# antoine311200/sow

Measured on AMD Instinct MI355X. Metric: SoWLinear fwd+bwd tokens/s, llama_60m rank=50 (56-layer SoWLinear stack), higher is better.
Workload: dtype bf16

## Files before the change

### sow_amd/csrc/api.hip

```cpp
#include "kernels.hpp"
#include <cstring>
#include <vector>
#include <cstdio>
#include <cstdlib>

namespace sow {

template <typename T, typename TO>
__global__ __launch_bounds__(256) void colsum_kernel(const T* M, int64_t ld, int64_t rows, int D, TO* out, float beta) {
  __shared__ float red[4][64];
  const int c = blockIdx.x * 64 + (threadIdx.x & 63), w = threadIdx.x >> 6;
  float s = 0.f;
  if (c < D)
    for (int64_t i = w; i < rows; i += 4) s += to_f32(M[i * ld + c]);
  red[w][threadIdx.x & 63] = s;
  __syncthreads();
  if (w == 0 && c < D) {
    float v = red[0][threadIdx.x] + red[1][threadIdx.x] + red[2][threadIdx.x] + red[3][threadIdx.x];
    if (beta != 0.f) v += beta * to_f32(out[c]);
    out[c] = from_f32<TO>(v);
  }
}
static int launch_colsum(const void* dy, int64_t T, int d_out, void* dbias, float beta, int dtype, int out_dtype,
                         hipStream_t stream) {
  const dim3 grid((d_out + 63) / 64);
  if (out_dtype != dtype && out_dtype != SOW_F32) return SOW_ERR_DTYPE;
  const bool o32 = out_dtype == SOW_F32;
  if (dtype == SOW_F32)
    hipLaunchKernelGGL((colsum_kernel<float, float>), grid, dim3(256), 0, stream, (const float*)dy, (int64_t)d_out, T, d_out, (float*)dbias, beta);
  else if (dtype == SOW_BF16 && o32)
    hipLaunchKernelGGL((colsum_kernel<bf16_t, float>), grid, dim3(256), 0, stream, (const bf16_t*)dy, (int64_t)d_out, T, d_out, (float*)dbias, beta);
  else if (dtype == SOW_BF16)
    hipLaunchKernelGGL((colsum_kernel<bf16_t, bf16_t>), grid, dim3(256), 0, stream, (const bf16_t*)dy, (int64_t)d_out, T, d_out, (bf16_t*)dbias, beta);
  else if (dtype == SOW_F16 && o32)
    hipLaunchKernelGGL((colsum_kernel<f16_t, float>), grid, dim3(256), 0, stream, (const f16_t*)dy, (int64_t)d_out, T, d_out, (float*)dbias, beta);
  else if (dtype == SOW_F16)
    hipLaunchKernelGGL((colsum_kernel<f16_t, f16_t>), grid, dim3(256), 0, stream, (const f16_t*)dy, (int64_t)d_out, T, d_out, (f16_t*)dbias, beta);
  else
    return SOW_ERR_DTYPE;
  SOW_CHECK_LAUNCH();
  return SOW_OK;
}
}

namespace sow {
static const char* const kSwitchNames[SW_COUNT] = {"FORCE_CHAIN_V1", "NO_SHORT_SPLIT", "NO_FUSED_H", "FORCE_GEMM_V1", "TN_NARROW",
                                                   "NO_GEMM3S",      "GEMM3S",         "GEMM3",      "NO_GROUPED",     "NO_PERSIST",     "NO_NT_STORE",    "NT_LOAD",        "NO_PAIR_FLUSH",  "F32_EXACT",
                                                   "NO_PARK16",      "TN_NO_NT_LOAD",  "NO_TN_ROWS",     "GEMM4",          "NO_GEMM4H",      "NO_CHAIN3F",     "NO_TN_F32Q",     "NO_SPLITK",
                                                   "NO_WIDE_CHAIN",  "NO_SHARED_X",    "NO_RAGGED",      "NO_RAGGED_GEMM", "NO_BLOCKED_QR",
                                                   "NO_SKINNY",      "NO_FUSED_ACC",   "NO_DEEP_ACC",    "NO_F16_TN",
                                                   "NO_ROW_ALIGN",   "NO_X_PAIR",      "NO_H_ROWS"};
static std::atomic<int> g_switch[SW_COUNT];
static std::once_flag g_switch_once;
static void switches_from_env() {
  for (int i = 0; i < SW_COUNT; ++i) {
    char name[64];
    snprintf(name, sizeof name, "SOW_AMD_%s", kSwitchNames[i]);
    const char* v = getenv(name);
    const bool tri = i == SW_GEMM3S || i == SW_GEMM3 || i == SW_GEMM4;
    const int on = i == SW_NO_ROW_ALIGN && v && v[0] >= '1' && v[0] <= '3' ? v[0] - '0' : 1;
    g_switch[i].store(!v ? -1 : (tri ? (v[0] != '0') : on), std::memory_order_relaxed);
  }
}
int sw(int which) {
  std::call_once(g_switch_once, switches_from_env);
  return g_switch[which].load(std::memory_order_relaxed);
}
}

using namespace sow;

static inline size_t al256(size_t v) { return (v + 255) & ~(size_t)255; }
static inline size_t esize(int dtype) { return dtype == SOW_F32 ? 4 : 2; }
static inline bool ok_dtype(int d) { return d == SOW_F32 || d == SOW_BF16 || d == SOW_F16; }
struct Dtype {
  int cd;
  bool param_f32;
  bool fuse;
  bool deep;
  bool native;
  bool native_bit;
  int perm() const { return (fuse ? SOW_FUSE_ACC : 0) | (deep ? SOW_FUSE_ACC_DEEP : 0); }
  bool layer_ok() const { return ok_dtype(cd) && !((param_f32 || native_bit) && cd == SOW_F32); }
};
static inline Dtype decode_dtype(int d) {
  Dtype f;
  f.cd = d & ~(SOW_FUSE_ACC | SOW_FUSE_ACC_DEEP | SOW_PARAM_F32 | SOW_ACC_NATIVE);
  f.param_f32 = (d & SOW_PARAM_F32) != 0;
  f.native_bit = (d & SOW_ACC_NATIVE) != 0;
  f.native = f.native_bit && f.param_f32;
  f.fuse = (d & SOW_FUSE_ACC) != 0 && !f.param_f32;
  f.deep = (d & SOW_FUSE_ACC_DEEP) != 0 && !f.param_f32;
  return f;
}
static inline bool flagged(int d) { return (d & (SOW_PARAM_F32 | SOW_ACC_NATIVE)) != 0; }
static inline int nofuse(int d) { return d & ~(SOW_FUSE_ACC | SOW_FUSE_ACC_DEEP); }

constexpr int SHORT_NTB = 128;
static inline int short_want(int ntb) { return ntb > 0 ? (256 + ntb - 1) / ntb : 1; }
static size_t short_hp_bytes(int64_t T, int d_in, int d_out, int r_live, int dtype) {
  const int ntb = ceil_div(T, 64);
  if (r_live > 64 || ntb <= 0 || ntb > SHORT_NTB) return 0;
  const int dmax = d_in > d_out ? d_in : d_out;
  int ks = short_want(ntb);
// ... 1529 lines not shown
```

### sow_amd/csrc/chain2.hip

```cpp
#include "kernels.hpp"
#include "lds_dma.hpp"

namespace sow {

#ifdef SOW_STAMPS
#define C2_STAMP(i)                                                                                  \
  do {                                                                                               \
    if (stamps && w == 0 && lane == 0) stamps[i] = __builtin_amdgcn_s_memrealtime();                \
  } while (0)
#else
#define C2_STAMP(i) \
  do {              \
  } while (0)
#endif
#ifdef SOW_STAMPS
#define C2_TICK() __builtin_amdgcn_s_memrealtime()
#define C2_ACC(var, t0) var += __builtin_amdgcn_s_memrealtime() - (t0)
#define C2_PUT(cond, i, var)                     \
  do {                                           \
    if (stamps && (cond) && lane == 0) stamps[i] = (var); \
  } while (0)
#else
#define C2_TICK() 0ull
#define C2_ACC(var, t0) (void)(t0)
#define C2_PUT(cond, i, var) \
  do {                       \
  } while (0)
#endif

constexpr int C2_NTG = 2;
constexpr int C2_NCW = 2 * C2_NTG;
constexpr int C2_NLW = 2;
constexpr int C2_BM = 32 * C2_NTG;
#ifndef C2_DEPTH_X
#define C2_DEPTH_X 4
#define C2_NSLOT_X 6
#define C2_AHEAD_X 5
#endif
constexpr int C2_DEPTH = C2_DEPTH_X;
constexpr int C2_STAGE = 4096;
constexpr int C2_NSLOT = C2_NSLOT_X;
constexpr int C2_AHEAD = C2_AHEAD_X;
#ifdef C2_EXPERIMENT_SHALLOW_X
static_assert(C2_NSLOT == C2_AHEAD + 1 && C2_NSLOT + C2_DEPTH == 10 && C2_DEPTH >= 3 && C2_DEPTH <= 6, "80 KiB");
#else
static_assert(C2_NSLOT == C2_AHEAD + 1 && C2_NSLOT + C2_DEPTH == 10 && C2_DEPTH >= 4 && C2_DEPTH <= 6,
              "80 KiB: 8 KiB per chunk slot + 2 x 4 KiB per X slot; two 8-KiB fp32 park tiles per token group must fit its X ring");
#endif
constexpr int C2_FSLOT = 8192;
constexpr int C2_LPW = 8 / C2_NLW;
constexpr int C2_RING0 = C2_NSLOT * C2_FSLOT;
constexpr int C2_RING = C2_DEPTH * C2_STAGE;
constexpr int C2_LDS = C2_RING0 + C2_NTG * C2_RING;
constexpr int C2_THREADS = 64 * (C2_NCW + C2_NLW);
constexpr int C2_RESIDENT = 512;


__host__ __device__ constexpr int c2_x_issued(int st, int nst, int depth, bool paired) {
  const int n = paired ? depth - 2 + 2 * ((st + 1) >> 1) : depth - 1 + st;
  return n < nst ? n : nst;
}

template <bool TR> __device__ __forceinline__ int img_chunk(int row, int c) {
  return TR ? (c ^ (((row >> 1) & 1) << 2)) : (c ^ ((row >> 1) & 7));
}

template <typename T, bool BWD, bool P16, bool AL>
__device__ __forceinline__ void chain2_block(const ChainParams& p, const int bid, char* smem, const int t, const int lane, const int w,
                                             uint64_t* stamps) {
  constexpr bool TR = !BWD;
  C2_STAMP(0);
  const int tb = p.ntb > 0 ? bid % p.ntb : bid;
  const int split = p.ntb > 0 ? bid / p.ntb : 0;
  const int64_t m0 = (int64_t)tb * C2_BM;
  const int D1 = p.D1, D2 = p.D2, rb = p.rb;
  const int nst_all = (D1 + 63) / 64, nsl_all = (D2 + 63) / 64;
  const int st0 = p.st_per > 0 ? split * p.st_per : 0;
  const int sl0 = p.sl_per > 0 ? split * p.sl_per : 0;
  const int nst = p.sl_per > 0 ? 0 : (p.st_per > 0 ? (nst_all - st0 < p.st_per ? nst_all - st0 : p.st_per) : nst_all);
  const int nsl = p.st_per > 0 ? 0 : (p.sl_per > 0 ? (nsl_all - sl0 < p.sl_per ? nsl_all - sl0 : p.sl_per) : nsl_all);
  const int total = nst + nsl;
  const T* Amat = (const T*)(BWD ? p.F2b : p.F1b);
  const T* Bmat = (const T*)(BWD ? p.F1b : p.F2b);
  const int64_t ldb = BWD ? p.ldf1b : p.ldf2b;
  const int rows_a = BWD ? D2 : D1, cols_b = BWD ? D1 : D2;
  const char* zp = zero_page_for(lane);
  const int ral = AL ? p.row_align : 0;

  if (w >= C2_NCW) {
    __builtin_amdgcn_s_setprio(3);
    const int lw = w - C2_NCW;
    const char* a_end = (const char*)(Amat + (int64_t)rows_a * rb);
    const bool own_last = rows_a > 0 && lw == ((rows_a - 1) & 63) / (8 * C2_LPW);
    uint32_t last_row_dw = 0u;
    if (own_last && lane < 32 && 2 * lane < rb) last_row_dw = *((const uint32_t*)(Amat + (int64_t)(rows_a - 1) * rb) + lane);
    asm volatile("" : "+v"(last_row_dw));
    auto chunk_is_a = [&](int c) { return BWD ? (c >= nst) : (c < nst); };
    const char* a_ptr[C2_LPW];
    const char* b_ptr[C2_LPW];
    int b_stride[C2_LPW], b_lc[C2_LPW];
#pragma unroll
    for (int ii = 0; ii < C2_LPW; ++ii) {
      const int i = C2_LPW * lw + ii;
      const int row = 8 * i + (lane >> 3), pc = lane & 7;
      const int lc = img_chunk<TR>(row, pc);
      a_ptr[ii] = (const char*)(Amat + (int64_t)row * rb) + 16 * lc;
      const bool bv = row < rb;
      b_ptr[ii] = bv ? (const char*)(Bmat + (int64_t)row * ldb + 8 * lc) : zp;
      b_stride[ii] = bv ? 128 : 0;
      b_lc[ii] = lc;
    }
    const int a_chunk_bytes = 128 * rb;
    const bool b_ragged = (cols_b & 63) != 0;
    const int nb_chunks = (cols_b + 63) / 64;
    auto issue = [&](int c) {
#ifdef C2_EXPERIMENT_NO_FACTOR_DMA
      if (c >= C2_NSLOT) return;
#endif
#ifdef C2_EXPERIMENT_HALF_FACTOR_DMA
      if (bid & 1) return;
#endif
      char* slot = smem + (c % C2_NSLOT) * C2_FSLOT;
      const int ci = c < nst ? st0 + c : sl0 + (c - nst);
      if (chunk_is_a(c)) {
#pragma unroll
        for (int ii = 0; ii < C2_LPW; ++ii) {
          const char* q = a_ptr[ii] + (int64_t)ci * a_chunk_bytes;
          dma16(q + 16 <= a_end ? (const void*)q : (const void*)zp, slot + (C2_LPW * lw + ii) * 1024);
        }
      } else {
#pragma unroll
        for (int ii = 0; ii < C2_LPW; ++ii) {
          const char* q = b_ptr[ii] + ci * b_stride[ii];
          if (b_ragged && ci == nb_chunks - 1 && ci * 64 + 8 * b_lc[ii] >= cols_b) q = zp;
          dma16((const void*)q, slot + (C2_LPW * lw + ii) * 1024);
        }
      }
    };
    const int ahead = ral ? C2_AHEAD - 1 : C2_AHEAD;
    const int pre = total < ahead ? total : ahead;
    for (int c = 0; c < pre; ++c) issue(c);
    uint64_t tw_dma = 0, tw_bar = 0;
    for (int c = 0; c < total; ++c) {
      const int newer = (total - 1 - c) < (ahead - 1) ? (total - 1 - c) : (ahead - 1);
      const uint64_t tk0 = C2_TICK();
      wait_groups<C2_LPW>(newer);
      C2_ACC(tw_dma, tk0);
      if (chunk_is_a(c)) {
        const int base = (c < nst ? st0 + c : sl0 + (c - nst)) * 64;
        const int lr = rows_a - 1 - base;
        if (own_last && lr >= 0 && lr < 64 && lane < 32) {
          const int cc = lane >> 2;
          *(uint32_t*)(smem + (c % C2_NSLOT) * C2_FSLOT + lr * 128 + img_chunk<TR>(lr, cc) * 16 + (lane & 3) * 4) = last_row_dw;
        }
      }
      if (c == nst) __builtin_amdgcn_s_setprio(0);
      if (c == nst) raw_barrier();
      const uint64_t tk1 = C2_TICK();
      raw_barrier();
      C2_ACC(tw_bar, tk1);
      if (c + ahead < total) issue(c + ahead);
    }
    C2_PUT(w == C2_NCW, 8, tw_dma);
    C2_PUT(w == C2_NCW, 9, tw_bar);
    if (nsl > 0) {
      raw_barrier();
    } else {
      raw_barrier();
    }
    raw_barrier();
    return;
  }

  if (p.pad_dst && bid * 64 < p.pad_rows) {
    const T* src = (const T*)p.pad_src;
    T* dst = (T*)p.pad_dst;
#pragma unroll
    for (int it = 0; it < 2; ++it) {
      const int idx = t + 256 * it, row = bid * 64 + (idx >> 3), c0 = (idx & 7) * 8;
      if (row < p.pad_rows) {
        u32x4 v;
        T* e = (T*)&v;
#pragma unroll
        for (int j = 0; j < 8; ++j) e[j] = (c0 + j < p.pad_r) ? src[(int64_t)row * p.pad_r + c0 + j] : (T)0.f;
        *(u32x4*)(dst + (int64_t)row * 64 + c0) = v;
      }
    }
  }
  const int tg = w & 1, hh = w >> 1;
  const int li = lane & 31, lh = lane >> 5;
  const int g = lane >> 4, jj = lane & 15, q = jj >> 2, pp = jj & 3;
  const int h2 = g >> 1;
  char* ring = smem + C2_RING0 + tg * C2_RING;
  const uint32_t ring_a = lds_addr(ring);
  const uint32_t slot_a = lds_addr(smem);
// ... 15 lines not shown
    xsrc[ii] = v ? (const char*)(X + tk * p.ldx + lc * 8 - xsh) : zp;
    xstride[ii] = v ? 128 : 0;
    xlc[ii] = lc;
  }
  const bool x_ragged = (D1 & 63) != 0;
  auto issue_x = [&](int st) {
    char* dst = ring + (st % C2_DEPTH) * C2_STAGE;
#pragma unroll
    for (int ii = 0; ii < 2; ++ii) {
      const char* qq = xsrc[ii] + (st0 + st) * xstride[ii];
      if constexpr (AL) {
        const int col = (st0 + st) * 64 + xlc[ii] * 8 - xsh;
        if ((x_ragged || xsh) && (col < 0 || col >= D1)) qq = zp;
      } else {
        if (x_ragged && (st0 + st) * 64 + xlc[ii] * 8 >= D1) qq = zp;
      }
      if (p.nt_load) dma16_nt((const void*)qq, dst + (2 * hh + ii) * 1024);
      else dma16((const void*)qq, dst + (2 * hh + ii) * 1024);
    }
  };

  const uint32_t xoff = (uint32_t)(li * 128);
  const int xsw = (li >> 1) & 7;
  uint32_t foff1[1], foff2;
  if constexpr (TR) {
    const int col = hh * 32 + 16 * (g & 1) + 4 * pp;
    const int r1 = 8 * h2 + q;
    foff1[0] = (uint32_t)(r1 * 128 + img_chunk<true>(r1, col >> 3) * 16 + (col & 7) * 2);
  } else {
    foff1[0] = (uint32_t)((hh * 32 + li) * 128);
  }
  const int ct = owr ? hh ^ 1 : hh;
  if constexpr (TR) {
    const int col = ct * 32 + 16 * (g & 1) + 4 * pp;
    const int r2 = 4 * h2 + q;
    foff2 = (uint32_t)(r2 * 128 + img_chunk<true>(r2, col >> 3) * 16 + (col & 7) * 2);
  } else {
    foff2 = (uint32_t)((ct * 32 + li) * 128 + 8 * lh);
  }

  f32x16 hacc;
#pragma unroll
  for (int i = 0; i < 16; ++i) hacc[i] = 0.f;

  const bool xpair = p.x_pair != 0;
  int issued = 0;
  for (const int pre = c2_x_issued(0, nst, C2_DEPTH, xpair); issued < pre; ++issued) issue_x(issued);

  uint64_t tw_x = 0, tw_b1 = 0, tw_b2 = 0;
#pragma unroll 1
  for (int st = 0; st < nst; ++st) {
    const int newer = issued - st - 1;
    const uint64_t tk0 = C2_TICK();
    wait_groups<2>(newer);
    C2_ACC(tw_x, tk0);
    const uint64_t tk1 = C2_TICK();
    raw_barrier();
    C2_ACC(tw_b1, tk1);
    if (st == 0) C2_STAMP(1);
    for (const int upto = c2_x_issued(st + 1, nst, C2_DEPTH, xpair); issued < upto; ++issued) issue_x(issued);
    const uint32_t xs = ring_a + (uint32_t)((st % C2_DEPTH) * C2_STAGE) + xoff;
    const uint32_t fs = slot_a + (uint32_t)((st % C2_NSLOT) * C2_FSLOT);
    const uint32_t fsp = AL && ord && st > 0 ? slot_a + (uint32_t)(((st - 1) % C2_NSLOT) * C2_FSLOT) : fs;
    u32x4 xf[4], ff[4];
#pragma unroll
    for (int ks = 0; ks < 4; ++ks) DS_READ_B128(xf[ks], xs + (uint32_t)(((2 * ks + lh) ^ xsw) * 16), 0);
    if constexpr (TR) {
      u32x2 bl[4], bh[4];
      if constexpr (AL) {
        const uint32_t b0 = fsp + foff1[0] + (ord ? 4096u : 0u);
        const uint32_t b1 = fs + foff1[0] + (ord ? 0u : 4096u);
        DS_READ_TR(bl[0], b0, 0);
        DS_READ_TR(bh[0], b0, 512);
        DS_READ_TR(bl[1], b0, 2048);
        DS_READ_TR(bh[1], b0, 2048 + 512);
        DS_READ_TR(bl[2], b1, 0);
        DS_READ_TR(bh[2], b1, 512);
        DS_READ_TR(bl[3], b1, 2048);
        DS_READ_TR(bh[3], b1, 2048 + 512);
      } else {
      const uint32_t b0 = fs + foff1[0];
      DS_READ_TR(bl[0], b0, 0);
      DS_READ_TR(bh[0], b0, 512);
      DS_READ_TR(bl[1], b0, 2048);
      DS_READ_TR(bh[1], b0, 2048 + 512);
      DS_READ_TR(bl[2], b0, 4096);
      DS_READ_TR(bh[2], b0, 4096 + 512);
      DS_READ_TR(bl[3], b0, 6144);
      DS_READ_TR(bh[3], b0, 6144 + 512);
      }
      LGKM_WAIT0();
#pragma unroll
      for (int ks = 0; ks < 4; ++ks) ff[ks] = join2(bl[ks], bh[ks]);
    } else {
#pragma unroll
      for (int ks = 0; ks < 4; ++ks) {
        if constexpr (AL) {
          const int kk = (ks + (ord ? 2 : 0)) & 3;
          DS_READ_B128(ff[ks], (ks < 2 ? fsp : fs) + foff1[0] + (uint32_t)(((2 * kk + lh) ^ xsw) * 16), 0);
        } else {
          DS_READ_B128(ff[ks], fs + foff1[0] + (uint32_t)(((2 * ks + lh) ^ xsw) * 16), 0);
        }
      }
      LGKM_WAIT0();
    }
    if constexpr (AL) {
      if (!(ord && st == 0)) {
// ... 50 lines not shown
#pragma unroll
        for (int rq = 0; rq < 4; ++rq) {
          u32x2 v = {pack16x2<T>(hv[4 * rq + 0], hv[4 * rq + 1]), pack16x2<T>(hv[4 * rq + 2], hv[4 * rq + 3])};
          if (hh == 1 && rq == 3 && lh == 1 && rb < 64) v[1] = (v[1] & 0xffffu) | (DT<T>::one_bits << 16);
          *(u32x2*)(img + (((hh * 4 + rq) ^ ((li >> 1) & 7)) * 16)) = v;
        }
      } else if (p.Hsave && tok < p.M) {
        T* Hs = (T*)p.Hsave + tok * 64 + hh * 32 + 4 * lh;
#pragma unroll
        for (int rq = 0; rq < 4; ++rq) {
          u32x2 v = {pack16x2<T>(hv[4 * rq + 0], hv[4 * rq + 1]), pack16x2<T>(hv[4 * rq + 2], hv[4 * rq + 3])};
          if (hh == 1 && rq == 3 && lh == 1 && rb < 64) v[1] = (v[1] & 0xffffu) | (DT<T>::one_bits << 16);
          *(u32x2*)(Hs + 8 * rq) = v;
        }
      }
    }
    char* xch = ring + (nst % C2_DEPTH) * C2_STAGE;
    *(u32x4*)(xch + hh * 2048 + lane * 16) = own[0];
    *(u32x4*)(xch + hh * 2048 + 1024 + lane * 16) = own[1];
    raw_barrier();
    u32x4 oth[2];
    const uint32_t pa = ring_a + (uint32_t)((nst % C2_DEPTH) * C2_STAGE + (hh ^ 1) * 2048 + lane * 16);
    DS_READ_B128(oth[0], pa, 0);
    DS_READ_B128(oth[1], pa, 1024);
    if (p.Hsave && p.h_rows && !p.Hpartial) {
      u32x4 hr[2];
      const uint32_t ia = ring_a + (uint32_t)(((nst + 1) % C2_DEPTH) * C2_STAGE);
#pragma unroll
      for (int pass = 0; pass < 2; ++pass) {
        const int r = 16 * hh + pass * 8 + (lane >> 3);
        DS_READ_B128(hr[pass], ia + (uint32_t)(r * 128 + (((lane & 7) ^ ((r >> 1) & 7)) * 16)), 0);
      }
      LGKM_WAIT0();
#pragma unroll
      for (int pass = 0; pass < 2; ++pass) {
        const int64_t tk = trow(16 * hh + pass * 8 + (lane >> 3));
        if (tk < p.M) {
          T* dst = (T*)p.Hsave + tk * 64 + (lane & 7) * 8;
          store_b128_nt(dst, hr[pass]);
        }
      }
    }
    LGKM_WAIT0();
    hf[0] = hh ? oth[0] : own[0], hf[1] = hh ? oth[1] : own[1];
    hf[2] = hh ? own[0] : oth[0], hf[3] = hh ? own[1] : oth[1];
  }
  C2_STAMP(3);
  T* Y = (T*)p.Y;
  const T* bias = (const T*)p.bias;
  const int ksteps = (rb + 15) / 16;
  auto tile_addr = [&](int buf, int row, int chunk) {
    return ring_a + (uint32_t)(buf * 8192 + row * 256 + ((chunk ^ (row & 15)) * 16));
  };
  const bool pairf = p.pair_flush != 0 && C2_RING >= 3 * 8192;
  auto flush = [&](int sl_prev) {
    const int buf = pairf ? sl_prev % 3 : (sl_prev & 1);
    u32x4 v0[2], v1[2];
#pragma unroll
    for (int pass = 0; pass < 2; ++pass) {
      const int r = 16 * hh + pass * 8 + (lane >> 3), c8 = lane & 7;
      DS_READ_B128(v0[pass], tile_addr(buf, r, 2 * c8), 0);
      DS_READ_B128(v1[pass], tile_addr(buf, r, 2 * c8 + 1), 0);
    }
    LGKM_WAIT0();
#pragma unroll
    for (int pass = 0; pass < 2; ++pass) {
      const int r = 16 * hh + pass * 8 + (lane >> 3), c8 = lane & 7;
      const int64_t tk = trow(r);
      const int col = (sl0 + sl_prev) * 64 + c8 * 8;
      if (tk < p.M && col < D2) {
        float v[8];
        const float* f0 = (const float*)&v0[pass];
        const float* f1 = (const float*)&v1[pass];
#pragma unroll
        for (int e = 0; e < 4; ++e) v[e] = f0[e], v[4 + e] = f1[e];
        T* dst = Y + tk * p.ldy + col;
        if (p.beta != 0.f) {
          const u32x4 old = *(const u32x4*)dst;
          const T* o = (const T*)&old;
#pragma unroll
          for (int e = 0; e < 8; ++e) v[e] += p.beta * (float)o[e];
        }
        if (bias) {
          const u32x4 bv = *(const u32x4*)(bias + col);
          const T* bb = (const T*)&bv;
#pragma unroll
          for (int e = 0; e < 8; ++e) v[e] += (float)bb[e];
        }
        const u32x4 ov = {pack16x2<T>(v[0], v[1]), pack16x2<T>(v[2], v[3]), pack16x2<T>(v[4], v[5]), pack16x2<T>(v[6], v[7])};
        if (p.nt_store) store_b128_nt(dst, ov);
        else *(u32x4*)dst = ov;
      }
    }
  };
  auto flush_pair = [&](int sl_a) {
#pragma unroll
    for (int half = 0; half < 2; ++half) {
      u32x4 v0[2], v1[2];
#pragma unroll
      for (int ps = 0; ps < 2; ++ps) {
        const int r = 16 * hh + (2 * half + ps) * 4 + (lane >> 4), c16 = lane & 15;
        const int buf = (sl_a + (c16 >> 3)) % 3, c8 = c16 & 7;
        DS_READ_B128(v0[ps], tile_addr(buf, r, 2 * c8), 0);
        DS_READ_B128(v1[ps], tile_addr(buf, r, 2 * c8 + 1), 0);
      }
      LGKM_WAIT0();
#pragma unroll
// ... 193 lines not shown
    *(u32x4*)(Hs + tok * 64 + c0) = (u32x4){pack16x2<T>(v[0], v[1]), pack16x2<T>(v[2], v[3]), pack16x2<T>(v[4], v[5]), pack16x2<T>(v[6], v[7])};
  } else {
    *(f32x4*)(Hs + tok * 64 + c0) = (f32x4){v[0], v[1], v[2], v[3]};
    *(f32x4*)(Hs + tok * 64 + c0 + 4) = (f32x4){v[4], v[5], v[6], v[7]};
  }
}

int launch_h_reduce(const float* Hpartial, int nsplit, void* Hsave, int64_t M, int rb, float scale, int dtype,
                    hipStream_t stream) {
  if (M <= 0) return SOW_OK;
  const dim3 grid((unsigned)((M * 8 + 255) / 256));
  if (dtype == SOW_BF16)
    hipLaunchKernelGGL(h_reduce_kernel<bf16_t>, grid, dim3(256), 0, stream, Hpartial, nsplit, (bf16_t*)Hsave, M, rb, scale);
  else if (dtype == SOW_F16)
    hipLaunchKernelGGL(h_reduce_kernel<f16_t>, grid, dim3(256), 0, stream, Hpartial, nsplit, (f16_t*)Hsave, M, rb, scale);
  else if (dtype == SOW_F32)
    hipLaunchKernelGGL(h_reduce_kernel<float>, grid, dim3(256), 0, stream, Hpartial, nsplit, (float*)Hsave, M, rb, scale);
  else
    return SOW_ERR_DTYPE;
  SOW_CHECK_LAUNCH();
  return SOW_OK;
}

void* g_chain2_stamps = nullptr;

static int chain2_grid(const ChainParams& p) {
  if (p.ntb > 0) {
    const int nsplit = p.st_per > 0 ? ceil_div((p.D1 + 63) / 64, p.st_per) : ceil_div((p.D2 + 63) / 64, p.sl_per);
    return p.ntb * nsplit;
  }
  return ceil_div(p.M, C2_BM);
}

int launch_chain2_group(const ChainParams* ps, int n, bool bwd, int dtype, hipStream_t stream) {
  if (n <= 0) return SOW_OK;
  if (dtype != SOW_BF16 && dtype != SOW_F16) return SOW_ERR_DTYPE;
  if (n > C2_MAXG) return SOW_ERR_SHAPE;
  ChainGroup g{};
  g.n = n;
  int64_t total = 0;
  for (int i = 0; i < n; ++i) {
    const ChainParams& p = ps[i];
    const void* Bp = bwd ? p.F1b : p.F2b;
    const int64_t ldB = bwd ? p.ldf1b : p.ldf2b;
    const void* Ap = bwd ? p.F2b : p.F1b;
    const int64_t ldA = bwd ? p.ldf2b : p.ldf1b;
    if ((reinterpret_cast<uintptr_t>(Bp) & 15) || ldB % 8 || (reinterpret_cast<uintptr_t>(Ap) & 3) || ldA != p.rb)
      return SOW_ERR_ALIGN;
    g.p[i] = p;
    g.p[i].nt_store = sw_on(SW_NO_NT_STORE) ? 0 : 1;
    g.p[i].nt_load = sw_on(SW_NT_LOAD) ? 1 : 0;
    g.p[i].h_rows = sw_on(SW_NO_H_ROWS) ? 0 : 1;
    g.p[i].x_pair = sw_on(SW_NO_X_PAIR) ? 0 : 1;
    g.p[i].pair_flush = sw_on(SW_NO_PAIR_FLUSH) ? 0 : 1;
    g.start[i] = (int)total;
    total += chain2_grid(p);
  }
  for (int i = n; i <= C2_MAXG; ++i) g.start[i] = (int)total;
  g.stamps = (uint64_t*)g_chain2_stamps;
  if (total <= 0) return SOW_OK;
  if (total > 0x7fffffff) return SOW_ERR_SHAPE;
  const int64_t grid = (sw_on(SW_NO_PERSIST) || total < C2_RESIDENT) ? total : C2_RESIDENT;
  bool p16 = !sw_on(SW_NO_PARK16);
  for (int i = 0; i < n; ++i) p16 = p16 && g.p[i].pair_flush && g.p[i].beta == 0.f && !g.p[i].bias;
  const int no_al = sw(SW_NO_ROW_ALIGN);
  bool al = false;
  for (int i = 0; i < n; ++i) {
    ChainParams& q = g.p[i];
    auto half_off = [](const void* base, int64_t ld, int D) {
      return ld % 64 == 32 && D % 64 > 0 && D % 64 <= 32 && (reinterpret_cast<uintptr_t>(base) & 127) == 0;
    };
    q.row_align = 0;
    if (q.ntb > 0) continue;
    if (no_al != 1 && no_al != 2 && half_off(q.X, q.ldx, q.D1)) q.row_align |= 1;
    if (no_al != 1 && no_al != 3 && p16 && half_off(q.Y, q.ldy, q.D2)) q.row_align |= 2;
    al = al || q.row_align != 0;
  }
#define C2_LAUNCH_AL(B, P, A)                                                                                        \
  do {                                                                                                               \
    if (dtype == SOW_F16) {                                                                                          \
      SOW_SET_MAX_LDS_ONCE(C2_LDS, (chain2_f16_kernel<B, P, A>));                                                    \
      hipLaunchKernelGGL((chain2_f16_kernel<B, P, A>), dim3((unsigned)grid), dim3(C2_THREADS), C2_LDS, stream, g);   \
    } else {                                                                                                         \
      SOW_SET_MAX_LDS_ONCE(C2_LDS, (chain2_kernel<B, P, A>));                                                        \
      hipLaunchKernelGGL((chain2_kernel<B, P, A>), dim3((unsigned)grid), dim3(C2_THREADS), C2_LDS, stream, g);       \
    }                                                                                                                \
  } while (0)
#define C2_LAUNCH(B, P)                \
  do {                                 \
    if (al) C2_LAUNCH_AL(B, P, true);  \
    else C2_LAUNCH_AL(B, P, false);    \
  } while (0)
  if (bwd) {
    if (p16) C2_LAUNCH(true, true);
    else C2_LAUNCH(true, false);
  } else {
    if (p16) C2_LAUNCH(false, true);
    else C2_LAUNCH(false, false);
  }
#undef C2_LAUNCH
#undef C2_LAUNCH_AL
  SOW_CHECK_LAUNCH();
  return SOW_OK;
}

int launch_chain2(const ChainParams& p, bool bwd, int dtype, hipStream_t stream) { return launch_chain2_group(&p, 1, bwd, dtype, stream); }

}

extern "C" int sow_debug_chain2_x_issued(int st, int nst, int depth, int paired) {
  return sow::c2_x_issued(st, nst, depth, paired != 0);
}
extern "C" int sow_debug_chain2_x_depth(void) { return sow::C2_DEPTH; }
```

### sow_amd/csrc/common.hpp

```cpp
#pragma once
#include <hip/hip_runtime.h>
#include <stdint.h>

#include <atomic>
#include <mutex>

#include "../../include/sow_amd.h"

namespace sow {

typedef __bf16 bf16_t;
typedef __attribute__((ext_vector_type(8))) __bf16 bf16x8;
typedef __attribute__((ext_vector_type(4))) __bf16 bf16x4;
typedef __attribute__((ext_vector_type(2))) __bf16 bf16x2;
typedef _Float16 f16_t;
typedef __attribute__((ext_vector_type(8))) _Float16 f16x8;
typedef __attribute__((ext_vector_type(2))) _Float16 f16x2;
typedef __attribute__((ext_vector_type(16))) float f32x16;
typedef __attribute__((ext_vector_type(4))) float f32x4;
typedef __attribute__((ext_vector_type(2))) float f32x2;
typedef __attribute__((ext_vector_type(4))) uint32_t u32x4;
typedef __attribute__((ext_vector_type(2))) uint32_t u32x2;

enum : int { SOW_F32 = 0, SOW_BF16 = 1, SOW_F16 = 2 };
// ... 98 lines not shown
}

inline int ceil_div(int64_t a, int64_t b) { return (int)((a + b - 1) / b); }

inline bool al16p(const void* p) { return (reinterpret_cast<uintptr_t>(p) & 15) == 0; }
inline bool al4p(const void* p) { return (reinterpret_cast<uintptr_t>(p) & 3) == 0; }

#define SOW_SET_MAX_LDS_ONCE(bytes, ...)                                                                            \
  do {                                                                                                              \
    static std::atomic<uint64_t> done__{0};                                                                         \
    int dev__ = 0;                                                                                                  \
    (void)hipGetDevice(&dev__);                                                                                     \
    const uint64_t bit__ = 1ull << (dev__ & 63);                                                                    \
    if (!(done__.load(std::memory_order_acquire) & bit__)) {                                                        \
      (void)hipFuncSetAttribute((const void*)(__VA_ARGS__), hipFuncAttributeMaxDynamicSharedMemorySize, (bytes));    \
      done__.fetch_or(bit__, std::memory_order_release);                                                            \
    }                                                                                                               \
  } while (0)

enum Switch : int {
  SW_FORCE_CHAIN_V1 = 0,
  SW_NO_SHORT_SPLIT,
  SW_NO_FUSED_H,
  SW_FORCE_GEMM_V1,
  SW_TN_NARROW,
  SW_NO_GEMM3S,
  SW_GEMM3S,
  SW_GEMM3,
  SW_NO_GROUPED,
  SW_NO_PERSIST,
  SW_NO_NT_STORE,
  SW_NT_LOAD,
  SW_NO_PAIR_FLUSH,
  SW_F32_EXACT,
  SW_NO_PARK16,
  SW_TN_NO_NT_LOAD,
  SW_NO_TN_ROWS,
  SW_GEMM4,
  SW_NO_GEMM4H,
  SW_NO_CHAIN3F,
  SW_NO_TN_F32Q,
  SW_NO_SPLITK,
  SW_NO_WIDE_CHAIN,
  SW_NO_SHARED_X,
  SW_NO_RAGGED,
  SW_NO_RAGGED_GEMM,
  SW_NO_BLOCKED_QR,
  SW_NO_SKINNY,
  SW_NO_FUSED_ACC,
  SW_NO_DEEP_ACC,
  SW_NO_F16_TN,
  SW_NO_ROW_ALIGN,
  SW_NO_X_PAIR,
  SW_NO_H_ROWS,
  SW_COUNT
};
int sw(int which);
inline bool sw_on(int which) { return sw(which) > 0; }

#ifdef SOW_GEMM_NO_NT
#define SOW_GEMM_NT(M) false
#else
#define SOW_GEMM_NT(M) ((M) >= 8192)
#endif

#define SOW_CHECK_LAUNCH()                     \
  do {                                         \
    hipError_t e__ = hipGetLastError();        \
    if (e__ != hipSuccess) return (int)e__;    \
  } while (0)

}
```

### sow_amd/csrc/kernels.hpp

```cpp
#pragma once
#include "common.hpp"

namespace sow {
struct ChainParams {
  const void* X;
  void* Y;
  const void *F1a, *F1b, *F2a, *F2b;
  void* Hsave;
  const void* bias;
  int64_t M, ldx, ldy, ldf1a, ldf1b, ldf2a, ldf2b;
  int D1, D2, ra, rb;
  float scale, beta;
  int fast_factors;
  const void* pad_src;
  void* pad_dst;
  int pad_rows, pad_r;
  int ntb, st_per, sl_per;
  float* Hpartial;
  const void* Hload;
  int nt_store;
  int nt_load;
  int h_rows;
  int pair_flush;
  int row_align;
  int x_pair;
  void* planes;
  size_t planes_bytes;
};
int launch_chain(ChainParams p, int dtype, bool bwd, hipStream_t stream);
constexpr int C2_MAXG = 4;
struct ChainGroup {
  ChainParams p[C2_MAXG];
  int start[C2_MAXG + 1];
  int n;
  uint64_t* stamps;
};
extern void* g_chain2_stamps;
bool chain2_supported(const ChainParams& p, int dtype);
int launch_chain2(const ChainParams& p, bool bwd, int dtype, hipStream_t stream);
int launch_chain2_group(const ChainParams* ps, int n, bool bwd, int dtype, hipStream_t stream);
bool chain2_shared_supported(const ChainParams* ps, int n, bool bwd, int dtype);
int launch_chain2_shared(const ChainParams* ps, int n, bool bwd, int dtype, hipStream_t stream);
int launch_h_reduce(const float* Hpartial, int nsplit, void* Hsave, int64_t M, int rb, float scale, int dtype,
                    hipStream_t stream);
bool chain2f_supported(const ChainParams& p, int dtype);
int launch_chain2f(const ChainParams& p, bool bwd, hipStream_t stream);
size_t chain3f_plane_bytes(int d_in, int d_out);
bool chain3f_supported(const ChainParams& p, int dtype);
int launch_chain3f(const ChainParams& p, bool bwd, hipStream_t stream);
struct TnJob {
  const void* M;
  const void* S;
  float* partial;
  int64_t ldm;
  int D;
  int ones_col;
  int ncg;
  int vec;
  int ones_col_in_s;
};
struct TnParams {
  TnJob job[2];
  int njobs;
  int64_t T;
  int ns;
  int slab_len;
};
struct ReduceJob {
  const float* partial;
  void* out;
  void* colsum;
  int64_t out_ld;
  int D, Dpad, r;
  int transpose;
  int ones_col;
  float alpha, beta;
  int ns;
};
// ... 265 lines not shown
```

### sow_amd/csrc/lds_dma.hpp

```cpp
#pragma once
#include "common.hpp"

namespace sow {

static __device__ __attribute__((aligned(256))) uint32_t g_zero_page[64];
__device__ __forceinline__ const char* zero_page_for(int lane) { return (const char*)(g_zero_page + (lane & 7) * 4); }

__device__ __forceinline__ uint32_t lds_addr(const void* p) {
  return (uint32_t)(uintptr_t)(__attribute__((address_space(3))) const char*)p;
}
#define DS_READ_B128(dst, addr, off) \
  asm volatile("ds_read_b128 %0, %1 offset:%2" : "=v"(dst) : "v"(addr), "n"(off) : "memory")
#define DS_READ_B64(dst, addr, off) \
  asm volatile("ds_read_b64 %0, %1 offset:%2" : "=v"(dst) : "v"(addr), "n"(off) : "memory")
#define DS_READ_B32(dst, addr, off) \
  asm volatile("ds_read_b32 %0, %1 offset:%2" : "=v"(dst) : "v"(addr), "n"(off) : "memory")
#define DS_READ_TR(dst, addr, off) \
  asm volatile("ds_read_b64_tr_b16 %0, %1 offset:%2" : "=v"(dst) : "v"(addr), "n"(off) : "memory")
#define LGKM_WAIT0()                                  \
  do {                                                \
    asm volatile("s_waitcnt lgkmcnt(0)" ::: "memory"); \
    __builtin_amdgcn_sched_barrier(0);                \
  } while (0)

__device__ __forceinline__ void raw_barrier() {
  asm volatile("s_waitcnt lgkmcnt(0)" ::: "memory");
  __builtin_amdgcn_s_barrier();
  __builtin_amdgcn_sched_barrier(0);
}
template <int PER> __device__ __forceinline__ void wait_groups(int newer) {
  switch (newer) {
    case 0: asm volatile("s_waitcnt vmcnt(0)" ::: "memory"); break;
    case 1: asm volatile("s_waitcnt vmcnt(%0)" ::"n"(PER) : "memory"); break;
    case 2: asm volatile("s_waitcnt vmcnt(%0)" ::"n"(2 * PER) : "memory"); break;
    case 3: asm volatile("s_waitcnt vmcnt(%0)" ::"n"(3 * PER) : "memory"); break;
    case 4: asm volatile("s_waitcnt vmcnt(%0)" ::"n"(4 * PER) : "memory"); break;
    default: asm volatile("s_waitcnt vmcnt(%0)" ::"n"(5 * PER) : "memory"); break;
  }
  __builtin_amdgcn_sched_barrier(0);
}
__device__ __forceinline__ void dma16(const void* src, char* lds_dst) {
  __builtin_amdgcn_global_load_lds((const __attribute__((address_space(1))) void*)src,
                                   (__attribute__((address_space(3))) void*)lds_dst, 16, 0, 0);
}
__device__ __forceinline__ void dma16_nt(const void* src, char* lds_dst) {
  __builtin_amdgcn_global_load_lds((const __attribute__((address_space(1))) void*)src,
                                   (__attribute__((address_space(3))) void*)lds_dst, 16, 0, 2);
}
__device__ __forceinline__ void store_b128_nt(void* dst, u32x4 v) {
  asm volatile("global_store_dwordx4 %0, %1, off nt\n\ts_nop 1" ::"v"(dst), "v"(v) : "memory");
}
__device__ __forceinline__ bf16x8 as_bf16x8(u32x4 v) { return __builtin_bit_cast(bf16x8, v); }
__device__ __forceinline__ u32x4 join2(u32x2 lo, u32x2 hi) { return (u32x4){lo[0], lo[1], hi[0], hi[1]}; }
__device__ __forceinline__ uint64_t pk_sub_f32(uint64_t a, uint64_t b) {
  uint64_t r;
  asm("v_pk_add_f32 %0, %1, %2 neg_lo:[0,1] neg_hi:[0,1]" : "=v"(r) : "v"(a), "v"(b));
  return r;
}
__device__ __forceinline__ void split3(float x0, float x1, uint32_t& h, uint32_t& m, uint32_t& l) {
  constexpr uint32_t HI = 0x07060302u;
  constexpr uint32_t MK = 0xffff0000u;
  const uint32_t u0 = __builtin_bit_cast(uint32_t, x0), u1 = __builtin_bit_cast(uint32_t, x1);
  h = __builtin_amdgcn_perm(u1, u0, HI);
  const uint64_t x64 = (uint64_t)u0 | ((uint64_t)u1 << 32);
  const uint64_t r64 = pk_sub_f32(x64, (uint64_t)(u0 & MK) | ((uint64_t)(u1 & MK) << 32));
  const uint32_t r0 = (uint32_t)r64, r1 = (uint32_t)(r64 >> 32);
  m = __builtin_amdgcn_perm(r1, r0, HI);
  const uint64_t q64 = pk_sub_f32(r64, (uint64_t)(r0 & MK) | ((uint64_t)(r1 & MK) << 32));
  l = __builtin_amdgcn_perm((uint32_t)(q64 >> 32), (uint32_t)q64, HI);
}
__device__ __forceinline__ void split3v(float x0, float x1, u32x4 (&pl)[3], int e) {
  uint32_t h, m, l;
  split3(x0, x1, h, m, l);
  pl[0][e] = h, pl[1][e] = m, pl[2][e] = l;
}
__device__ __forceinline__ f32x16 mfma_x3(const u32x4 (&a)[3], const u32x4 (&b)[3], f32x16 acc) {
  acc = mfma32(as_bf16x8(a[2]), as_bf16x8(b[0]), acc);
  acc = mfma32(as_bf16x8(a[0]), as_bf16x8(b[2]), acc);
  acc = mfma32(as_bf16x8(a[1]), as_bf16x8(b[1]), acc);
  acc = mfma32(as_bf16x8(a[1]), as_bf16x8(b[0]), acc);
  acc = mfma32(as_bf16x8(a[0]), as_bf16x8(b[1]), acc);
  acc = mfma32(as_bf16x8(a[0]), as_bf16x8(b[0]), acc);
  return acc;
}

}
```

Baseline: 9.094 million.

## Stage factor chunks through loader-wave registers instead of direct LDS DMA

Adds a default-on path in the chain2 kernel where the loader waves fetch factor chunks with global_load_dwordx4 into rotating register groups and write them into the LDS ring with ds_write_b128. The first few chunks still use direct LDS DMA. A new schedule function decides which register group serves each chunk and how long to wait on it, and the last-row patch is applied with an explicit LDS write. The aim is deeper prefetch without extra LDS slots and fewer stalls from the global-to-LDS DMA path. In exchange the loader waves use more VGPRs and the vmcnt bookkeeping is more complex. The change also hard-disables the paired fp32 flush and widens the X wait helper.

```diff
diff --git a/sow_amd/csrc/api.hip b/sow_amd/csrc/api.hip
--- a/sow_amd/csrc/api.hip
+++ b/sow_amd/csrc/api.hip
@@ -49,7 +49,7 @@
                                                    "NO_PARK16",      "TN_NO_NT_LOAD",  "NO_TN_ROWS",     "GEMM4",          "NO_GEMM4H",      "NO_CHAIN3F",     "NO_TN_F32Q",     "NO_SPLITK",
                                                    "NO_WIDE_CHAIN",  "NO_SHARED_X",    "NO_RAGGED",      "NO_RAGGED_GEMM", "NO_BLOCKED_QR",
                                                    "NO_SKINNY",      "NO_FUSED_ACC",   "NO_DEEP_ACC",    "NO_F16_TN",
-                                                   "NO_ROW_ALIGN",   "NO_X_PAIR",      "NO_H_ROWS"};
+                                                   "NO_ROW_ALIGN",   "NO_X_PAIR",      "NO_FACTOR_STAGE", "NO_H_ROWS"};
 static std::atomic<int> g_switch[SW_COUNT];
 static std::once_flag g_switch_once;
 static void switches_from_env() {
diff --git a/sow_amd/csrc/chain2.hip b/sow_amd/csrc/chain2.hip
--- a/sow_amd/csrc/chain2.hip
+++ b/sow_amd/csrc/chain2.hip
@@ -37,16 +37,22 @@
 #define C2_NSLOT_X 6
 #define C2_AHEAD_X 5
 #endif
+#ifndef C2_FSTAGE_R_X
+#define C2_FSTAGE_R_X 4
+#endif
 constexpr int C2_DEPTH = C2_DEPTH_X;
 constexpr int C2_STAGE = 4096;
 constexpr int C2_NSLOT = C2_NSLOT_X;
 constexpr int C2_AHEAD = C2_AHEAD_X;
+constexpr int C2_FSTAGE_R = C2_FSTAGE_R_X;
 #ifdef C2_EXPERIMENT_SHALLOW_X
-static_assert(C2_NSLOT == C2_AHEAD + 1 && C2_NSLOT + C2_DEPTH == 10 && C2_DEPTH >= 3 && C2_DEPTH <= 6, "80 KiB");
+static_assert(C2_NSLOT == C2_AHEAD + 1 && C2_NSLOT + C2_DEPTH == 10 && C2_DEPTH >= 3 && C2_DEPTH <= 7, "80 KiB");
 #else
-static_assert(C2_NSLOT == C2_AHEAD + 1 && C2_NSLOT + C2_DEPTH == 10 && C2_DEPTH >= 4 && C2_DEPTH <= 6,
-              "80 KiB: 8 KiB per chunk slot + 2 x 4 KiB per X slot; two 8-KiB fp32 park tiles per token group must fit its X ring");
+static_assert(C2_NSLOT == C2_AHEAD + 1 && C2_NSLOT + C2_DEPTH == 10 && C2_DEPTH >= 4 && C2_DEPTH <= 7 && C2_NSLOT >= 3,
+              "80 KiB: 8 KiB per chunk slot + 2 x 4 KiB per X slot; two 8-KiB fp32 park tiles per token group must fit its X ring; "
+              "row alignment keeps chunk c - 1 alive through step c, so the ring needs 3 slots");
 #endif
+static_assert(C2_FSTAGE_R == 3 || C2_FSTAGE_R == 4, "register groups of a loader wave: 16 VGPRs each");
 constexpr int C2_FSLOT = 8192;
 constexpr int C2_LPW = 8 / C2_NLW;
 constexpr int C2_RING0 = C2_NSLOT * C2_FSLOT;
@@ -59,6 +65,20 @@
 __host__ __device__ constexpr int c2_x_issued(int st, int nst, int depth, bool paired) {
   const int n = paired ? depth - 2 + 2 * ((st + 1) >> 1) : depth - 1 + st;
   return n < nst ? n : nst;
+}
+
+struct C2FactorSched {
+  int group;
+  int load_after;
+  int write_after;
+  int slot;
+  int wait;
+};
+__host__ __device__ constexpr C2FactorSched c2_factor_sched(int k, int total, int nslot, int R, bool aligned) {
+  const int ahead = aligned ? nslot - 2 : nslot - 1;
+  const int rest = total - 1 - k;
+  if (k < ahead) return {-1, -1, -1, k % nslot, rest < ahead + R - 1 ? rest : ahead + R - 1};
+  return {(k - ahead) % R, k - ahead - R < 0 ? -1 : k - ahead - R, k - ahead, k % nslot, rest < R - 1 ? rest : R - 1};
 }
 
 template <bool TR> __device__ __forceinline__ int img_chunk(int row, int c) {
@@ -96,51 +116,106 @@
     if (own_last && lane < 32 && 2 * lane < rb) last_row_dw = *((const uint32_t*)(Amat + (int64_t)(rows_a - 1) * rb) + lane);
     asm volatile("" : "+v"(last_row_dw));
     auto chunk_is_a = [&](int c) { return BWD ? (c >= nst) : (c < nst); };
-    const char* a_ptr[C2_LPW];
-    const char* b_ptr[C2_LPW];
-    int b_stride[C2_LPW], b_lc[C2_LPW];
-#pragma unroll
-    for (int ii = 0; ii < C2_LPW; ++ii) {
-      const int i = C2_LPW * lw + ii;
-      const int row = 8 * i + (lane >> 3), pc = lane & 7;
-      const int lc = img_chunk<TR>(row, pc);
-      a_ptr[ii] = (const char*)(Amat + (int64_t)row * rb) + 16 * lc;
-      const bool bv = row < rb;
-      b_ptr[ii] = bv ? (const char*)(Bmat + (int64_t)row * ldb + 8 * lc) : zp;
-      b_stride[ii] = bv ? 128 : 0;
-      b_lc[ii] = lc;
-    }
+    const int row0 = 8 * C2_LPW * lw + (lane >> 3);
+    int lc16[C2_LPW];
+#pragma unroll
+    for (int ii = 0; ii < C2_LPW; ++ii) lc16[ii] = 16 * img_chunk<TR>(row0 + 8 * ii, lane & 7);
+    const int a_row0 = row0 * 2 * rb;
+    const int64_t b_row0 = (int64_t)row0 * ldb * 2;
     const int a_chunk_bytes = 128 * rb;
     const bool b_ragged = (cols_b & 63) != 0;
     const int nb_chunks = (cols_b + 63) / 64;
-    auto issue = [&](int c) {
+    auto src_of = [&](int c, int ii) -> const char* {
+      const int ci = c < nst ? st0 + c : sl0 + (c - nst);
+      if (chunk_is_a(c)) {
+        const char* q = (const char*)Amat + ((int64_t)ci * a_chunk_bytes + ii * 16 * rb) + (a_row0 + lc16[ii]);
+        return q + 16 <= a_end ? q : zp;
+      }
+      const char* q = (const char*)Bmat + ((int64_t)ci * 128 + (int64_t)ii * 16 * ldb) + (b_row0 + lc16[ii]);
+      bool ok = row0 + 8 * ii < rb;
+      if (b_ragged && ci == nb_chunks - 1 && ci * 64 + (lc16[ii] >> 1) >= cols_b) ok = false;
+      return ok ? q : zp;
+    };
+    auto skipped = [&](int c) -> bool {
 #ifdef C2_EXPERIMENT_NO_FACTOR_DMA
-      if (c >= C2_NSLOT) return;
+      if (c >= C2_NSLOT) return true;
 #endif
 #ifdef C2_EXPERIMENT_HALF_FACTOR_DMA
-      if (bid & 1) return;
+      if ((bid >> 3) & 1) return true;
 #endif
+      return false;
+    };
+    auto issue = [&](int c) {
+      if (skipped(c)) return;
       char* slot = smem + (c % C2_NSLOT) * C2_FSLOT;
-      const int ci = c < nst ? st0 + c : sl0 + (c - nst);
-      if (chunk_is_a(c)) {
-#pragma unroll
-        for (int ii = 0; ii < C2_LPW; ++ii) {
-          const char* q = a_ptr[ii] + (int64_t)ci * a_chunk_bytes;
-          dma16(q + 16 <= a_end ? (const void*)q : (const void*)zp, slot + (C2_LPW * lw + ii) * 1024);
-        }
-      } else {
-#pragma unroll
-        for (int ii = 0; ii < C2_LPW; ++ii) {
-          const char* q = b_ptr[ii] + ci * b_stride[ii];
-          if (b_ragged && ci == nb_chunks - 1 && ci * 64 + 8 * b_lc[ii] >= cols_b) q = zp;
-          dma16((const void*)q, slot + (C2_LPW * lw + ii) * 1024);
-        }
-      }
+#pragma unroll
+      for (int ii = 0; ii < C2_LPW; ++ii) dma16((const void*)src_of(c, ii), slot + (C2_LPW * lw + ii) * 1024);
     };
     const int ahead = ral ? C2_AHEAD - 1 : C2_AHEAD;
     const int pre = total < ahead ? total : ahead;
     for (int c = 0; c < pre; ++c) issue(c);
     uint64_t tw_dma = 0, tw_bar = 0;
+    if (p.fstage) {
+      static_assert(C2_LPW == 4, "a register group is four 16-byte pieces per lane");
+      constexpr int R = C2_FSTAGE_R;
+      RegGroup rg[R];
+      const uint32_t wr_a = lds_addr(smem) + (uint32_t)(C2_LPW * lw * 1024 + lane * 16);
+      auto sched = [&](int k) { return c2_factor_sched(k, total, C2_NSLOT, R, ral != 0); };
+      auto load = [&](RegGroup& g, int k) {
+        if (skipped(k)) return;
+#pragma unroll
+        for (int ii = 0; ii < C2_LPW; ++ii) {
+          const char* q = src_of(k, ii);
+          GLOAD_B128(g.v[ii], q);
+        }
+      };
+      auto fix_last_row = [&](int k) {
+        if (!chunk_is_a(k)) return;
+        const int base = (k < nst ? st0 + k : sl0 + (k - nst)) * 64;
+        const int lr = rows_a - 1 - base;
+        if (own_last && lr >= 0 && lr < 64 && lane < 32) {
+          const int cc = lane >> 2;
+          const uint32_t a = lds_addr(smem) + (uint32_t)((k % C2_NSLOT) * C2_FSLOT + lr * 128 + img_chunk<TR>(lr, cc) * 16 + (lane & 3) * 4);
+          DS_WRITE_B32(a, last_row_dw);
+        }
+      };
+      auto step = [&](RegGroup& g, int c, bool tail) {
+        const C2FactorSched s = sched(c);
+        if (s.group < 0) {
+          const uint64_t tk0 = C2_TICK();
+          wait_groups8<C2_LPW>(s.wait);
+          C2_ACC(tw_dma, tk0);
+          fix_last_row(c);
+        }
+        if (c == nst) __builtin_amdgcn_s_setprio(0);
+        if (c == nst) raw_barrier();
+        const uint64_t tk1 = C2_TICK();
+        raw_barrier();
+        C2_ACC(tw_bar, tk1);
+        const int k = c + ahead;
+        if (k < total) {
+          const C2FactorSched wr = sched(k);
+          const uint64_t tk2 = C2_TICK();
+          wait_reg_group(g, wr.wait);
+          C2_ACC(tw_dma, tk2);
+          write_reg_group(g, wr_a + (uint32_t)(wr.slot * C2_FSLOT));
+          fix_last_row(k);
+          if (!tail && k + R < total) load(g, k + R);
+        }
+      };
+#pragma unroll
+      for (int j = 0; j < R; ++j)
+        if (ahead + j < total) load(rg[j], ahead + j);
+      int c = 0;
+#pragma unroll 1
+      for (; c + R <= total; c += R) {
+#pragma unroll
+        for (int j = 0; j < R; ++j) step(rg[j], c + j, false);
+      }
+#pragma unroll
+      for (int j = 0; j < R - 1; ++j)
+        if (c + j < total) step(rg[j], c + j, true);
+    } else
     for (int c = 0; c < total; ++c) {
       const int newer = (total - 1 - c) < (ahead - 1) ? (total - 1 - c) : (ahead - 1);
       const uint64_t tk0 = C2_TICK();
@@ -262,7 +337,7 @@
   for (int st = 0; st < nst; ++st) {
     const int newer = issued - st - 1;
     const uint64_t tk0 = C2_TICK();
-    wait_groups<2>(newer);
+    wait_groups8<2>(newer);
     C2_ACC(tw_x, tk0);
     const uint64_t tk1 = C2_TICK();
     raw_barrier();
@@ -419,7 +494,8 @@
   auto tile_addr = [&](int buf, int row, int chunk) {
     return ring_a + (uint32_t)(buf * 8192 + row * 256 + ((chunk ^ (row & 15)) * 16));
   };
-  const bool pairf = p.pair_flush != 0 && C2_RING >= 3 * 8192;
+  constexpr bool C2_PAIR_F32 = false;
+  const bool pairf = C2_PAIR_F32 && p.pair_flush != 0 && C2_RING >= 3 * 8192;
   auto flush = [&](int sl_prev) {
     const int buf = pairf ? sl_prev % 3 : (sl_prev & 1);
     u32x4 v0[2], v1[2];
@@ -719,6 +795,7 @@
     g.p[i].nt_load = sw_on(SW_NT_LOAD) ? 1 : 0;
     g.p[i].h_rows = sw_on(SW_NO_H_ROWS) ? 0 : 1;
     g.p[i].x_pair = sw_on(SW_NO_X_PAIR) ? 0 : 1;
+    g.p[i].fstage = sw_on(SW_NO_FACTOR_STAGE) ? 0 : 1;
     g.p[i].pair_flush = sw_on(SW_NO_PAIR_FLUSH) ? 0 : 1;
     g.start[i] = (int)total;
     total += chain2_grid(p);
@@ -779,3 +856,9 @@
   return sow::c2_x_issued(st, nst, depth, paired != 0);
 }
 extern "C" int sow_debug_chain2_x_depth(void) { return sow::C2_DEPTH; }
+extern "C" void sow_debug_chain2_factor_sched(int k, int total, int nslot, int groups, int aligned, int* out) {
+  const sow::C2FactorSched s = sow::c2_factor_sched(k, total, nslot, groups, aligned != 0);
+  out[0] = s.group, out[1] = s.load_after, out[2] = s.write_after, out[3] = s.slot, out[4] = s.wait;
+}
+extern "C" int sow_debug_chain2_factor_slots(void) { return sow::C2_NSLOT; }
+extern "C" int sow_debug_chain2_factor_groups(void) { return sow::C2_FSTAGE_R; }
diff --git a/sow_amd/csrc/common.hpp b/sow_amd/csrc/common.hpp
--- a/sow_amd/csrc/common.hpp
+++ b/sow_amd/csrc/common.hpp
@@ -174,6 +174,7 @@
   SW_NO_F16_TN,
   SW_NO_ROW_ALIGN,
   SW_NO_X_PAIR,
+  SW_NO_FACTOR_STAGE,
   SW_NO_H_ROWS,
   SW_COUNT
 };
diff --git a/sow_amd/csrc/kernels.hpp b/sow_amd/csrc/kernels.hpp
--- a/sow_amd/csrc/kernels.hpp
+++ b/sow_amd/csrc/kernels.hpp
@@ -24,6 +24,7 @@
   int pair_flush;
   int row_align;
   int x_pair;
+  int fstage;
   void* planes;
   size_t planes_bytes;
 };
diff --git a/sow_amd/csrc/lds_dma.hpp b/sow_amd/csrc/lds_dma.hpp
--- a/sow_amd/csrc/lds_dma.hpp
+++ b/sow_amd/csrc/lds_dma.hpp
@@ -38,6 +38,44 @@
     default: asm volatile("s_waitcnt vmcnt(%0)" ::"n"(5 * PER) : "memory"); break;
   }
   __builtin_amdgcn_sched_barrier(0);
+}
+template <int PER> __device__ __forceinline__ void wait_groups8(int newer) {
+  switch (newer) {
+    case 0: asm volatile("s_waitcnt vmcnt(0)" ::: "memory"); break;
+    case 1: asm volatile("s_waitcnt vmcnt(%0)" ::"n"(PER) : "memory"); break;
+    case 2: asm volatile("s_waitcnt vmcnt(%0)" ::"n"(2 * PER) : "memory"); break;
+    case 3: asm volatile("s_waitcnt vmcnt(%0)" ::"n"(3 * PER) : "memory"); break;
+    case 4: asm volatile("s_waitcnt vmcnt(%0)" ::"n"(4 * PER) : "memory"); break;
+    case 5: asm volatile("s_waitcnt vmcnt(%0)" ::"n"(5 * PER) : "memory"); break;
+    case 6: asm volatile("s_waitcnt vmcnt(%0)" ::"n"(6 * PER) : "memory"); break;
+    case 7: asm volatile("s_waitcnt vmcnt(%0)" ::"n"(7 * PER) : "memory"); break;
+    default: asm volatile("s_waitcnt vmcnt(%0)" ::"n"(8 * PER) : "memory"); break;
+  }
+  __builtin_amdgcn_sched_barrier(0);
+}
+struct RegGroup {
+  u32x4 v[4];
+};
+#define GLOAD_B128(dst, ptr) asm volatile("global_load_dwordx4 %0, %1, off" : "=v"(dst) : "v"(ptr) : "memory")
+#define DS_WRITE_B128(addr, src, off) asm volatile("ds_write_b128 %0, %1 offset:%2" ::"v"(addr), "v"(src), "n"(off) : "memory")
+#define DS_WRITE_B32(addr, src) asm volatile("ds_write_b32 %0, %1" ::"v"(addr), "v"(src) : "memory")
+__device__ __forceinline__ void wait_reg_group(RegGroup& g, int newer) {
+  switch (newer) {
+    case 0: asm volatile("s_waitcnt vmcnt(0)" ::: "memory"); break;
+    case 1: asm volatile("s_waitcnt vmcnt(4)" ::: "memory"); break;
+    case 2: asm volatile("s_waitcnt vmcnt(8)" ::: "memory"); break;
+    case 3: asm volatile("s_waitcnt vmcnt(12)" ::: "memory"); break;
+    default: asm volatile("s_waitcnt vmcnt(16)" ::: "memory"); break;
+  }
+  __builtin_amdgcn_sched_barrier(0);
+  asm volatile("" : "+v"(g.v[0]), "+v"(g.v[1]), "+v"(g.v[2]), "+v"(g.v[3])::"memory");
+  __builtin_amdgcn_sched_barrier(0);
+}
+__device__ __forceinline__ void write_reg_group(const RegGroup& g, uint32_t lds_a) {
+  DS_WRITE_B128(lds_a, g.v[0], 0);
+  DS_WRITE_B128(lds_a, g.v[1], 1024);
+  DS_WRITE_B128(lds_a, g.v[2], 2048);
+  DS_WRITE_B128(lds_a, g.v[3], 3072);
 }
 __device__ __forceinline__ void dma16(const void* src, char* lds_dst) {
   __builtin_amdgcn_global_load_lds((const __attribute__((address_space(1))) void*)src,
```

Result: slower. 8.667 million (-4.7%).
